# enkeejunior1/Diffusion-Pullback

Measured on AMD Instinct MI355X. Metric: pullback top-k SVD iters/sec (SD-v1.5 mid-block, 4x64x64), higher is better.
Workload: dtype bf16; 1 GPU; BASELINE configs[2]: SD-v1.5 4x64x64 latent, no edit prompt (seeded null ctx[1,77,768]), mid-block h[1280,8,8], t=696.27; pca_rank=5, ctx=null, samples_total=5, samples_this_rank=5, samples_advanced_together=1, spectrum=shaped (configs.Spectrum()), parallelism=single process, no collective, rccl_world_size=0, repeats=7

## Files before the change

diffusion_pullback_amd/csrc/attn_fused.hip:

```cpp
#include "kernels.h"

namespace dpb {

#ifndef DPB_ATT_ABL
#define DPB_ATT_ABL 0
#endif
#ifndef DPB_OUT_STORE_ATT
#define DPB_OUT_STORE_ATT 0
#endif
#define DPB_ATT_PAD 8

constexpr int att_waves(int d) { return d > 80 ? 4 : 8; }

template <int D, int W = att_waves(D)> struct FA {
  static constexpr int WAVES = W, NT = WAVES * 64;
  static constexpr int NS = (D + 15) / 16;
  static constexpr int DP = NS * 16;
  static constexpr int ND = (D + 31) / 32;
  static constexpr int DO = ND * 32;
  static constexpr int BI = D <= 80 ? 128 : 64;
  static constexpr int LDR = (DP > DO ? DP : DO) + DPB_ATT_PAD;
  static constexpr int LDT = BI + 4;
  static constexpr int ROW_ELEMS = BI * LDR;
  static constexpr int T_ELEMS = DO * LDT;
// ... 14 lines not shown
}
template <int D, int NTH = FA<D>::NT>
__device__ inline void commit_row(const RowRegs<D, NTH>& rg, bf16* lds, int tid) {
  using F = FA<D>;
  constexpr int CPR = F::DP / 8, N = (F::BI * CPR + NTH - 1) / NTH;
#pragma unroll
  for (int i = 0; i < N; ++i) {
    const int c = tid + i * NTH;
    if (c < F::BI * CPR) *reinterpret_cast<uint4*>(lds + (c / CPR) * F::LDR + (c % CPR) * 8) = rg.v[i];
  }
}
template <int D, int NTH = FA<D>::NT> struct TRegs { uint4 v[(FA<D>::DO * (FA<D>::BI / 8) + NTH - 1) / NTH]; };
template <int D, int NTH = FA<D>::NT>
__device__ inline void fetch_t(const bf16* __restrict__ src, long gs, TRegs<D, NTH>& rg, int tid) {
  using F = FA<D>;
  constexpr int CPR = F::BI / 8, N = (F::DO * CPR + NTH - 1) / NTH;
#pragma unroll
  for (int i = 0; i < N; ++i) {
    const int c = tid + i * NTH;
    const int r = c / CPR, cc = (c % CPR) * 8;
    rg.v[i] = make_uint4(0, 0, 0, 0);
    if (c < F::DO * CPR && r < D) rg.v[i] = *reinterpret_cast<const uint4*>(src + (long)r * gs + cc);
  }
}
template <int D, int NTH = FA<D>::NT>
__device__ inline void commit_t(const TRegs<D, NTH>& rg, bf16* lds, int tid) {
  using F = FA<D>;
  constexpr int CPR = F::BI / 8, N = (F::DO * CPR + NTH - 1) / NTH;
#pragma unroll
  for (int i = 0; i < N; ++i) {
    const int c = tid + i * NTH;
    if (c < F::DO * CPR) {
      bf16* dst = lds + (c / CPR) * F::LDT + (c % CPR) * 8;
      *reinterpret_cast<uint2*>(dst) = make_uint2(rg.v[i].x, rg.v[i].y);
      *reinterpret_cast<uint2*>(dst + 4) = make_uint2(rg.v[i].z, rg.v[i].w);
    }
  }
}
template <int D>
__device__ inline void load_outer_frags(const bf16* __restrict__ rowptr, bf16x8* f, int lhi) {
  using F = FA<D>;
#pragma unroll
  for (int st = 0; st < F::NS; ++st) {
    const int col = st * 16 + lhi * 8;
    uint4 v = make_uint4(0, 0, 0, 0);
    if (col < D) v = *reinterpret_cast<const uint4*>(rowptr + col);
    f[st] = *reinterpret_cast<bf16x8*>(&v);
  }
}
__device__ inline bf16x8 lds_a_frag(const bf16* tile, int row, int ld, int col) {
  return *reinterpret_cast<const bf16x8*>(tile + row * ld + col);
}
__device__ inline bf16x8 lds_t_frag(const bf16* tile, int drow, int ld, int base, int lhi) {
  uint2 lo = *reinterpret_cast<const uint2*>(tile + drow * ld + base + 4 * lhi);
  uint2 hi = *reinterpret_cast<const uint2*>(tile + drow * ld + base + 8 + 4 * lhi);
  uint4 v = make_uint4(lo.x, lo.y, hi.x, hi.y);
  return *reinterpret_cast<bf16x8*>(&v);
}
typedef __attribute__((ext_vector_type(4))) short short4_;
__device__ inline bf16x8 lds_tr_frag(const bf16* tile, int ld, int base, int d0, int lane) {
  const int i16 = lane & 15, g = lane >> 4;
  const bf16* p = tile + (base + 4 * (g >> 1) + (i16 >> 2)) * ld + d0 + (g & 1) * 16 + (i16 & 3) * 4;
  short4_ lo = __builtin_amdgcn_ds_read_tr16_b64_v4i16((__attribute__((address_space(3))) short4_*)p);
  short4_ hi = __builtin_amdgcn_ds_read_tr16_b64_v4i16((__attribute__((address_space(3))) short4_*)(p + 8 * ld));
  uint2 l2 = *reinterpret_cast<uint2*>(&lo), h2 = *reinterpret_cast<uint2*>(&hi);
  uint4 v = make_uint4(l2.x, l2.y, h2.x, h2.y);
  return *reinterpret_cast<bf16x8*>(&v);
}
template <int FL>
__device__ inline void pack_b(const float* x, bf16x8* out) {
  out[0] = H16<FL>::pack8(x);
  out[1] = H16<FL>::pack8(x + 8);
}
struct BlockXY { int x, y; };
__device__ inline BlockXY xcd_group_blocks(int on) {
  const int nx = gridDim.x, ny = gridDim.y;
  if (!on || (ny & 7)) return {(int)blockIdx.x, (int)blockIdx.y};
  const int lin = blockIdx.y * nx + blockIdx.x, xcd = lin & 7, slot = lin >> 3;
  return {slot % nx, (slot / nx) * 8 + xcd};
}

static int g_attn_shared = getenv("DPB_ATTN_SHARED") ? atoi(getenv("DPB_ATTN_SHARED")) : 2;
void attn_debug_shared(int bits) { g_attn_shared = bits; }

#define MFMA(a, b, c) H16<FL>::mfma(a, b, c)

struct FusedArgs {
  const bf16 *Q, *K, *V, *O;
  const bf16 *KT, *VT, *QT;
  const float* stats;
  float* Drow;
  float* Dout;
  const bf16 *dQ, *dK, *dV, *dVT;
  bf16* dO;
  const bf16 *gO, *gOT;
  bf16 *gQ, *gK, *gV;
  int accQ, accK, accV;
  int xcd;
  int L, C, Co, H, kps;
  float scale;
};

template <int D, int FL, int W = att_waves(D)>
__global__ __launch_bounds__((FA<D, W>::NT)) void attn_fwd_kernel(FusedArgs a, bf16* O, float* stats_out) {
  using F = FA<D, W>;
  __shared__ __attribute__((aligned(16))) bf16 sm[2 * F::ROW_ELEMS];
  bf16* sK = sm; bf16* sV = sK + F::ROW_ELEMS;
  const int tid = threadIdx.x, lane = tid & 63, wave = tid >> 6, l31 = lane & 31, lhi = lane >> 5;
  const BlockXY blk = xcd_group_blocks(a.xcd);
  const int b = blk.y / a.H, h = blk.y % a.H;
  const int q_ = blk.x * (F::WAVES * 32) + wave * 32 + l31;
  const bool live = q_ < a.L;
  const int q = live ? q_ : a.L - 1;
  const long LC = (long)a.L * a.C;
  const bf16* Kp = a.K + b * LC + h * D;
  const bf16* Vp = a.V + b * LC + h * D;
  bf16x8 qf[F::NS];
  load_outer_frags<D>(a.Q + b * LC + (long)q * a.C + h * D, qf, lhi);
  const float c2 = a.scale * 1.44269504088896f;
  constexpr float FWD_THR = 4.f;
  constexpr bool LSUM = F::DP > D;
  constexpr unsigned ONE16 = FL ? 0x3C00u : 0x3F80u, VONE = LSUM ? ONE16 : 0u;
  f32x16 acc[F::ND];
#pragma unroll
  for (int d = 0; d < F::ND; ++d)
#pragma unroll
    for (int r = 0; r < 16; ++r) acc[d][r] = 0.f;
  float m = -INFINITY, l = 0.f;
  RowRegs<D, F::NT> rK, rV;
  fetch_row<D, F::NT>(Kp, a.C, rK, tid); fetch_row<D, F::NT, VONE>(Vp, a.C, rV, tid);
  for (int k0 = 0; k0 < a.L; k0 += F::BI) {
    __syncthreads();
    commit_row<D, F::NT>(rK, sK, tid); commit_row<D, F::NT>(rV, sV, tid);
    __syncthreads();
    if (k0 + F::BI < a.L) {
      const int k1 = k0 + F::BI;
      fetch_row<D, F::NT>(Kp + (long)k1 * a.C, a.C, rK, tid); fetch_row<D, F::NT, VONE>(Vp + (long)k1 * a.C, a.C, rV, tid);
    }
#pragma unroll
    for (int kb = 0; kb < F::BI / 32; ++kb) {
      f32x16 s;
#pragma unroll
      for (int r = 0; r < 16; ++r) s[r] = 0.f;
#pragma unroll
      for (int stp = 0; stp < F::NS; ++stp) s = MFMA(lds_a_frag(sK, kb * 32 + l31, F::LDR, stp * 16 + lhi * 8), qf[stp], s);
      float mx = s[0];
#pragma unroll
      for (int r = 1; r < 16; ++r) mx = fmaxf(mx, s[r]);
      mx = fmaxf(mx, __shfl_xor(mx, 32, 64)) * c2;
      if (!__all(mx - m <= FWD_THR)) {
        const float mn = fmaxf(m, mx);
        const float alpha = __builtin_amdgcn_exp2f(m - mn);
#pragma unroll
        for (int d = 0; d < F::ND; ++d)
#pragma unroll
          for (int r = 0; r < 16; ++r) acc[d][r] *= alpha;
        if (!LSUM) l *= alpha;
        m = mn;
      }
      float p[16];
#pragma unroll
      for (int r = 0; r < 16; ++r) p[r] = __builtin_amdgcn_exp2f(__builtin_fmaf(s[r], c2, -m));
      if (!LSUM) {
        float ps = 0.f;
#pragma unroll
        for (int r = 0; r < 16; ++r) ps += p[r];
// ... 92 lines not shown
        kf[stp] = lds_a_frag(sK, kb * 32 + l31, F::LDR, stp * 16 + lhi * 8);
        dkf[stp] = lds_a_frag(sdK, kb * 32 + l31, F::LDR, stp * 16 + lhi * 8);
      }
    };
    if constexpr (PIPE) load1(0);
#pragma unroll
    for (int kb = 0; kb < F::BI / 32; ++kb) {
      bf16x8 vf[2][F::ND], dvf[2][F::ND];
      if constexpr (PIPE) {
#pragma unroll
        for (int ks = 0; ks < 2; ++ks)
#pragma unroll
          for (int d = 0; d < F::ND; ++d) {
            vf[ks][d] = lds_tr_frag(sV, F::LDR, kb * 32 + ks * 16, d * 32, lane);
            dvf[ks][d] = lds_tr_frag(sdV, F::LDR, kb * 32 + ks * 16, d * 32, lane);
          }
        __builtin_amdgcn_sched_barrier(0);
      } else {
        load1(kb);
      }
      f32x16 s, ds;
#pragma unroll
      for (int r = 0; r < 16; ++r) s[r] = ds[r] = 0.f;
#pragma unroll
      for (int stp = 0; stp < F::NS; ++stp) {
        s = MFMA(kf[stp], qf[stp], s);
        ds = MFMA(kf[stp], dqf[stp], ds);
        if (!((DPB_ATT_ABL & 2) && D == 40 && stp == F::NS - 1)) ds = MFMA(dkf[stp], qf[stp], ds);
      }
      if constexpr (PIPE) {
        __builtin_amdgcn_sched_barrier(0);
        if (kb + 1 < F::BI / 32) load1(kb + 1);
        __builtin_amdgcn_sched_barrier(0);
      }
      float p[16], x[16];
#pragma unroll
      for (int r = 0; r < 16; ++r) {
        p[r] = (DPB_ATT_ABL & 4) ? c2 * s[r] - m2 : __builtin_amdgcn_exp2f(c2 * s[r] - m2);
        x[r] = p[r] * (a.scale * ds[r]);
        if constexpr (!SUMROW) delta += x[r];
      }
      bf16x8 pb[2], xb[2];
      pack_b<FL>(p, pb);
      pack_b<FL>(x, xb);
#pragma unroll
      for (int ks = 0; ks < 2; ++ks)
#pragma unroll
        for (int d = 0; d < F::ND; ++d) {
          if constexpr (!PIPE) {
            vf[ks][d] = lds_tr_frag(sV, F::LDR, kb * 32 + ks * 16, d * 32, lane);
            dvf[ks][d] = lds_tr_frag(sdV, F::LDR, kb * 32 + ks * 16, d * 32, lane);
          }
          if ((DPB_ATT_ABL & 1) && D == 40 && ks == 1 && d == 1) continue;
          acc[d] = MFMA(vf[ks][d], xb[ks], acc[d]);
          acc[d] = MFMA(dvf[ks][d], pb[ks], acc[d]);
        }
    }
  }
  if constexpr (SUMROW) delta = __shfl(acc[D / 32][((D % 32) & 3) + 4 * ((D % 32) >> 3)], l31, 64);
  else delta += __shfl_xor(delta, 32, 64);
  const long LCo = (long)a.L * a.Co;
  const bf16* Op = a.O + b * LCo + (long)q * a.Co + h * D;
  bf16* dOp = a.dO + j * LCo + (long)q * a.Co + h * D;
#pragma unroll
  for (int d = 0; d < F::ND; ++d)
#pragma unroll
    for (int g = 0; g < 4; ++g) {
      const int col = d * 32 + 8 * g + 4 * lhi;
      if (col < D && live) {
        uint2 ov = *reinterpret_cast<const uint2*>(Op + col);
        unsigned ow[2] = {ov.x, ov.y};
        unsigned w[2];
#pragma unroll
        for (int i = 0; i < 2; ++i) {
          float o0 = H16<FL>::lo(ow[i]), o1 = H16<FL>::hi(ow[i]);
          float v0 = acc[d][g * 4 + 2 * i] - delta * o0, v1 = acc[d][g * 4 + 2 * i + 1] - delta * o1;
          w[i] = H16<FL>::pack2(v0, v1);
        }
        store_out8<DPB_OUT_STORE_ATT>(dOp + col, w[0], w[1]);
      }
    }
}

template <int D, int FL>
__global__ __launch_bounds__(FA<D>::NT) void attn_adj_q_kernel(FusedArgs a) {
  using F = FA<D>;
  __shared__ __attribute__((aligned(16))) bf16 sm[2 * F::ROW_ELEMS];
  bf16* sK = sm; bf16* sV = sK + F::ROW_ELEMS;
  const int tid = threadIdx.x, lane = tid & 63, wave = tid >> 6, l31 = lane & 31, lhi = lane >> 5;
  const BlockXY blk = xcd_group_blocks(a.xcd);
  const int j = blk.y / a.H, h = blk.y % a.H, b = j / a.kps;
  const int q_ = blk.x * (F::WAVES * 32) + wave * 32 + l31;
  const bool live = q_ < a.L;
  const int q = live ? q_ : a.L - 1;
  const long LC = (long)a.L * a.C;
  const bf16* Kp = a.K + b * LC + h * D;
  const bf16* Vp = a.V + b * LC + h * D;
  bf16x8 qf[F::NS], gof[F::NS], of[F::NS];
  load_outer_frags<D>(a.Q + b * LC + (long)q * a.C + h * D, qf, lhi);
  const long LCo = (long)a.L * a.Co;
  load_outer_frags<D>(a.gO + j * LCo + (long)q * a.Co + h * D, gof, lhi);
  load_outer_frags<D>(a.O + b * LCo + (long)q * a.Co + h * D, of, lhi);
  float Dq = 0.f;
#pragma unroll
  for (int stp = 0; stp < F::NS; ++stp) {
    const unsigned short* g16 = reinterpret_cast<const unsigned short*>(&gof[stp]);
    const unsigned short* o16 = reinterpret_cast<const unsigned short*>(&of[stp]);
#pragma unroll
    for (int e = 0; e < 8; ++e) Dq += H16<FL>::up(g16[e]) * H16<FL>::up(o16[e]);
  }
  Dq += __shfl_xor(Dq, 32, 64);
  const float* st = a.stats + (((long)b * a.H + h) * a.L + q) * 2;
  const float c2 = a.scale * 1.44269504088896f;
  const float m2 = st[0] * 1.44269504088896f - __builtin_log2f(st[1]);
  f32x16 acc[F::ND];
#pragma unroll
  for (int d = 0; d < F::ND; ++d)
#pragma unroll
    for (int r = 0; r < 16; ++r) acc[d][r] = 0.f;
  RowRegs<D> rK, rV;
  fetch_row<D>(Kp, a.C, rK, tid); fetch_row<D>(Vp, a.C, rV, tid);
  for (int k0 = 0; k0 < a.L; k0 += F::BI) {
    __syncthreads();
    commit_row<D>(rK, sK, tid); commit_row<D>(rV, sV, tid);
    __syncthreads();
    if (k0 + F::BI < a.L) {
      const int k1 = k0 + F::BI;
      fetch_row<D>(Kp + (long)k1 * a.C, a.C, rK, tid); fetch_row<D>(Vp + (long)k1 * a.C, a.C, rV, tid);
    }
#pragma unroll
    for (int kb = 0; kb < F::BI / 32; ++kb) {
      f32x16 s, gp;
#pragma unroll
      for (int r = 0; r < 16; ++r) s[r] = gp[r] = 0.f;
#pragma unroll
      for (int stp = 0; stp < F::NS; ++stp) {
        s = MFMA(lds_a_frag(sK, kb * 32 + l31, F::LDR, stp * 16 + lhi * 8), qf[stp], s);
        gp = MFMA(lds_a_frag(sV, kb * 32 + l31, F::LDR, stp * 16 + lhi * 8), gof[stp], gp);
      }
      float gs[16];
#pragma unroll
      for (int r = 0; r < 16; ++r) gs[r] = __builtin_amdgcn_exp2f(c2 * s[r] - m2) * (gp[r] - Dq);
      bf16x8 gsb[2];
      pack_b<FL>(gs, gsb);
#pragma unroll
      for (int ks = 0; ks < 2; ++ks)
#pragma unroll
        for (int d = 0; d < F::ND; ++d)
          acc[d] = MFMA(lds_tr_frag(sK, F::LDR, kb * 32 + ks * 16, d * 32, lane), gsb[ks], acc[d]);
    }
  }
  bf16* gQp = a.gQ + j * LC + (long)q * a.C + h * D;
#pragma unroll
  for (int d = 0; d < F::ND; ++d)
#pragma unroll
    for (int g = 0; g < 4; ++g) {
      const int col = d * 32 + 8 * g + 4 * lhi;
      if (col < D && live) {
        float v[4];
#pragma unroll
        for (int i = 0; i < 4; ++i) v[i] = a.scale * acc[d][g * 4 + i];
        if (a.accQ) {
          uint2 ov = *reinterpret_cast<const uint2*>(gQp + col);
          v[0] += H16<FL>::lo(ov.x); v[1] += H16<FL>::hi(ov.x);
          v[2] += H16<FL>::lo(ov.y); v[3] += H16<FL>::hi(ov.y);
        }
// ... 611 lines not shown
}

static bool head_dim_ok(int d) { return d == 40 || d == 64 || d == 80 || d == 160; }
#define DPB_ATT_DISPATCH(d, fl, ...)                                                        \
  do {                                                                                       \
    if ((fl) == 0) { constexpr int FL = 0; DPB_ATT_D(d, __VA_ARGS__) } else { constexpr int FL = 1; DPB_ATT_D(d, __VA_ARGS__) } \
  } while (0)
#define DPB_ATT_D(d, ...)                                          \
  if ((d) == 40) { constexpr int D = 40; __VA_ARGS__; }            \
  else if ((d) == 64) { constexpr int D = 64; __VA_ARGS__; }       \
  else if ((d) == 80) { constexpr int D = 80; __VA_ARGS__; }       \
  else { constexpr int D = 160; __VA_ARGS__; }

int cross_attention_supported(int dtype, int d, int Lq, int Lk, int kv_const) {
  return dtype != DT_F32 && kv_const && head_dim_ok(d) && Lk <= XKEYS && Lq % 32 == 0 && (Lq >= 128 ? Lq % 128 == 0 : true);
}

int launch_attn_cross(const CrossAttnArgs& f, int nt, hipStream_t st) {
  CrossArgs a;
  a.Q = (const bf16*)f.Q; a.K = (const bf16*)f.K; a.V = (const bf16*)f.V; a.BT = (const bf16*)f.BT;
  a.X = (const bf16*)f.X; a.Y = (bf16*)f.Y;
  a.L = f.L; a.Lk = f.Lk; a.Lkp = f.Lkp; a.C = f.C; a.Ck = f.Ck; a.Cx = f.Cx; a.Cy = f.Cy; a.H = f.H; a.kps = f.kps;
  a.a_is_v = f.adjoint; a.accumulate = f.accumulate; a.scale = f.scale; a.xcd = 0;
  a.c_in = f.adjoint ? 1.f : f.scale; a.c_out = f.adjoint ? f.scale : 1.f;
  a.primal = f.primal; a.Pst = f.primal ? f.Pstash : nullptr;
  if (f.primal) { a.a_is_v = 0; a.c_in = 1.f; a.c_out = 1.f; a.accumulate = 0; }
  const int waves = f.L >= 128 ? 4 : f.L / 32;
  dim3 grid(f.L / (waves * 32), nt * f.H);
  if (!head_dim_ok(f.d)) { set_error("cross attention: head dim %d unsupported", f.d); return -1; }
  if (a.Pst) DPB_ATT_DISPATCH(f.d, f.fl, DPB_LAUNCH((attn_cross_kernel<D, FL, true>), grid, dim3(waves * 64), 0, st, a));
  else DPB_ATT_DISPATCH(f.d, f.fl, DPB_LAUNCH((attn_cross_kernel<D, FL>), grid, dim3(waves * 64), 0, st, a));
  DPB_CHECK(hipGetLastError());
  return 0;
}

int fused_attention_supported(int dtype, int d, int L, int kv_const) {
  return dtype != DT_F32 && !kv_const && head_dim_ok(d) && ((L >= 256 && L % (att_waves(d) * 32) == 0) || (d == 160 && L == 64));
}

static int attn_xcd_on() { static int on = getenv("DPB_ATTN_XCD") ? atoi(getenv("DPB_ATTN_XCD")) : 0; return on; }

static FusedArgs to_args(const FusedAttnArgs& f) {
  FusedArgs a;
  a.xcd = attn_xcd_on();
  a.Q = (const bf16*)f.Q; a.K = (const bf16*)f.K; a.V = (const bf16*)f.V; a.O = (const bf16*)f.O;
  a.KT = (const bf16*)f.KT; a.VT = (const bf16*)f.VT; a.QT = (const bf16*)f.QT; a.stats = f.stats; a.Drow = f.Drow; a.Dout = nullptr;
  a.dQ = (const bf16*)f.dQ; a.dK = (const bf16*)f.dK; a.dV = (const bf16*)f.dV; a.dVT = (const bf16*)f.dVT; a.dO = (bf16*)f.dO;
  a.gO = (const bf16*)f.gO; a.gOT = (const bf16*)f.gOT; a.gQ = (bf16*)f.gQ; a.gK = (bf16*)f.gK; a.gV = (bf16*)f.gV;
  a.accQ = f.accQ; a.accK = f.accK; a.accV = f.accV;
  a.L = f.L; a.C = f.C; a.Co = f.Co; a.H = f.H; a.kps = f.kps; a.scale = f.scale;
  return a;
}

int launch_attn_fwd_fused(const FusedAttnArgs& f, int batch, void* O, float* stats, hipStream_t st) {
  FusedArgs a = to_args(f);
  dim3 grid((f.L + att_waves(f.d) * 32 - 1) / (att_waves(f.d) * 32), batch * f.H);
  if (!head_dim_ok(f.d)) { set_error("fused attention: head dim %d unsupported", f.d); return -1; }
  static const int fwd4 = getenv("DPB_ATTN_FWD4") ? atoi(getenv("DPB_ATTN_FWD4")) : 1;
  if (fwd4 && att_waves(f.d) == 8 && f.L % 128 == 0 && f.L >= 256 && (long)grid.x * grid.y < 256) {
    dim3 g4(f.L / 128, batch * f.H);
    if (f.d == 40) { if (f.fl) DPB_LAUNCH((attn_fwd_kernel<40, 1, 4>), g4, dim3(256), 0, st, a, (bf16*)O, stats); else DPB_LAUNCH((attn_fwd_kernel<40, 0, 4>), g4, dim3(256), 0, st, a, (bf16*)O, stats); }
    else if (f.d == 64) { if (f.fl) DPB_LAUNCH((attn_fwd_kernel<64, 1, 4>), g4, dim3(256), 0, st, a, (bf16*)O, stats); else DPB_LAUNCH((attn_fwd_kernel<64, 0, 4>), g4, dim3(256), 0, st, a, (bf16*)O, stats); }
    else { if (f.fl) DPB_LAUNCH((attn_fwd_kernel<80, 1, 4>), g4, dim3(256), 0, st, a, (bf16*)O, stats); else DPB_LAUNCH((attn_fwd_kernel<80, 0, 4>), g4, dim3(256), 0, st, a, (bf16*)O, stats); }
    DPB_CHECK(hipGetLastError());
    return 0;
  }
  DPB_ATT_DISPATCH(f.d, f.fl, DPB_LAUNCH((attn_fwd_kernel<D, FL>), grid, dim3(att_waves(D) * 64), 0, st, a, (bf16*)O, stats));
  DPB_CHECK(hipGetLastError());
  return 0;
}

static int att_block_waves(int d, int L, int pairs) {
  static const int force = getenv("DPB_ATTN_WAVES") ? atoi(getenv("DPB_ATTN_WAVES")) : 0;
  if (d != 40 || L % 256) return att_waves(d);
  if (force == 4 || force == 8) return force;
  return ((long)(L / 256) * pairs) % 256 == 0 ? 8 : 4;
}

int attn_jvp_block_waves(int d, int L, int pairs) { return att_block_waves(d, L, pairs); }

int launch_attn_jvp_fused(const FusedAttnArgs& f, int nt, hipStream_t st) {
  FusedArgs a = to_args(f);
  if (!head_dim_ok(f.d)) { set_error("fused attention: head dim %d unsupported", f.d); return -1; }
  if (att_block_waves(f.d, f.L, nt * f.H) == 4 && f.d == 40) {
    dim3 g4(f.L / 128, nt * f.H);
    if (f.fl) DPB_LAUNCH((attn_jvp_kernel<40, 1, 4>), g4, dim3(256), 0, st, a);
    else DPB_LAUNCH((attn_jvp_kernel<40, 0, 4>), g4, dim3(256), 0, st, a);
    DPB_CHECK(hipGetLastError());
    return 0;
  }
  dim3 grid((f.L + att_waves(f.d) * 32 - 1) / (att_waves(f.d) * 32), nt * f.H);
  DPB_ATT_DISPATCH(f.d, f.fl, DPB_LAUNCH((attn_jvp_kernel<D, FL>), grid, dim3(att_waves(D) * 64), 0, st, a));
  DPB_CHECK(hipGetLastError());
  return 0;
}

static int attn_adj_route(int d, int L, int kps, int nt, bool have_drow) {
  static const int multi = getenv("DPB_ATTN_MULTI") ? atoi(getenv("DPB_ATTN_MULTI")) : 1;
  const int shared = g_attn_shared;
  const bool dsh = d == 40 || (d == 64 && (shared & 4));
  int r = 0;
  if (dsh && (multi & 1) && L % 128 == 0 && nt % kps == 0) r |= 1;
  if (dsh && (shared & 2) && L % 64 == 0 && kps >= 4 && nt % kps == 0 && have_drow) r |= 2;
  return r;
}
int attn_adj_route_bits(int d, int L, int kps, int nt) { return attn_adj_route(d, L, kps, nt, true); }

int launch_attn_adj_fused(const FusedAttnArgs& f, int nt, hipStream_t st) {
  FusedArgs a = to_args(f);
  dim3 grid((f.L + att_waves(f.d) * 32 - 1) / (att_waves(f.d) * 32), nt * f.H);
  if (!head_dim_ok(f.d)) { set_error("fused attention: head dim %d unsupported", f.d); return -1; }
  const int route = attn_adj_route(f.d, f.L, f.kps, nt, f.Drow != nullptr);
  if (route & 1) {
    constexpr int TJ = 5;
    const int ngrp = (f.kps + TJ - 1) / TJ;
    const dim3 gq(f.L / 128, (nt / f.kps) * f.H * ngrp);
    if (route & 2) a.Dout = a.Drow;
#define DPB_ADJQ(DV, FLV) DPB_LAUNCH((attn_adj_q_multi_kernel<DV, TJ, FLV>), gq, dim3(256), 0, st, a)
    if (f.d == 40) { if (f.fl) DPB_ADJQ(40, 1); else DPB_ADJQ(40, 0); }
    else { if (f.fl) DPB_ADJQ(64, 1); else DPB_ADJQ(64, 0); }
#undef DPB_ADJQ
  } else {
    DPB_ATT_DISPATCH(f.d, f.fl, DPB_LAUNCH((attn_adj_q_kernel<D, FL>), grid, dim3(att_waves(D) * 64), 0, st, a));
  }
  if (route & 2) {
    constexpr int TJ = 5;
    const int ngrp = (f.kps + TJ - 1) / TJ;
    const dim3 gs(f.L / 64, (nt / f.kps) * f.H * ngrp);
    const unsigned nrd = (unsigned)(((long)nt * f.L * f.H + 255) / 256);
#define DPB_ADJKV(DV, FLV)                                                                                                          \
    do {                                                                                                                              \
      if (!(route & 1)) DPB_LAUNCH((attn_rowdot_kernel<DV, FLV>), dim3(nrd), dim3(256), 0, st, a, nt);                              \
      DPB_LAUNCH((attn_adj_kv_shared_kernel<DV, TJ, FLV>), gs, dim3(SHK<DV, TJ>::NT), 0, st, a);                                    \
    } while (0)
    if (f.d == 40) { if (f.fl) DPB_ADJKV(40, 1); else DPB_ADJKV(40, 0); }
    else { if (f.fl) DPB_ADJKV(64, 1); else DPB_ADJKV(64, 0); }
#undef DPB_ADJKV
  } else if (att_block_waves(f.d, f.L, nt * f.H) == 4 && f.d == 40) {
    dim3 g4(f.L / 128, nt * f.H);
    if (f.fl) DPB_LAUNCH((attn_adj_kv_kernel<40, 1, 4>), g4, dim3(256), 0, st, a);
    else DPB_LAUNCH((attn_adj_kv_kernel<40, 0, 4>), g4, dim3(256), 0, st, a);
  } else {
    DPB_ATT_DISPATCH(f.d, f.fl, DPB_LAUNCH((attn_adj_kv_kernel<D, FL>), grid, dim3(att_waves(D) * 64), 0, st, a));
  }
  DPB_CHECK(hipGetLastError());
  return 0;
}

}
```

diffusion_pullback_amd/csrc/engine.cpp:

```cpp
#include <math.h>
#include <stdarg.h>
#include <stdio.h>
#include <stdlib.h>
#include <string.h>

#include <string>
#include <vector>

#include "../../include/dpb.h"
#include "kernels.h"

namespace dpb {

static thread_local char g_err[1024] = "";
void set_error(const char* fmt, ...) {
  va_list ap;
  va_start(ap, fmt);
  vsnprintf(g_err, sizeof(g_err), fmt, ap);
  va_end(ap);
}
const char* last_error() { return g_err; }
thread_local long launch_count = 0;

static inline size_t align_up(size_t v, size_t a = 256) { return (v + a - 1) / a * a; }
// ... 1732 lines not shown
int dpb_engine_profile(dpb_engine* e, int enable) {
  if (!e) return fail("null engine");
  for (auto& p : e->prof) { (void)hipEventDestroy(p.a); (void)hipEventDestroy(p.b); }
  e->prof.clear();
  e->profiling = enable != 0;
  if (e->profiling) {
    hipEvent_t a, b;
    DPB_CHECK(hipEventCreate(&a));
    DPB_CHECK(hipEventCreate(&b));
    float best = 1e9f;
    for (int i = 0; i < 24; ++i) {
      DPB_CHECK(hipEventRecord(a, e->stream));
      if (int r = launch_axpy(e->dtype, e->ws + e->zeros, e->ws + e->zeros, 64, 0, e->stream)) return r;
      DPB_CHECK(hipEventRecord(b, e->stream));
      DPB_CHECK(hipEventSynchronize(b));
      float ms = 0;
      DPB_CHECK(hipEventElapsedTime(&ms, a, b));
      if (i >= 4) best = ms < best ? ms : best;
    }
    (void)hipEventDestroy(a);
    (void)hipEventDestroy(b);
    best -= 1.5e-3f;
    if (best < 0.f) best = 0.f;
    e->prof_overhead_ms = best < 1e8f ? best : 0.f;
  }
  return 0;
}

int dpb_engine_profile_dump(dpb_engine* e, const char* path) {
  if (!e || !path) return fail("null argument");
  DPB_CHECK(hipStreamSynchronize(e->stream));
  FILE* f = fopen(path, "w");
  if (!f) return fail("cannot open %s", path);
  fprintf(f, "idx,big,gather,M,N,K,Z,us,tflops,raw_us,bracket_overhead_us\n");
  int i = 0;
  for (auto& p : e->prof) {
    float raw = 0;
    (void)hipEventElapsedTime(&raw, p.a, p.b);
    const float ms = raw > e->prof_overhead_ms ? raw - e->prof_overhead_ms : 0.f;
    fprintf(f, "%d,%d,%d,%d,%d,%d,%d,%.2f,%.2f,%.2f,%.2f\n", i++, p.big, p.gather, p.M, p.N, p.K, p.Z, ms * 1e3, ms > 0 ? p.flops / (ms * 1e-3) / 1e12 : 0.0,
            raw * 1e3, e->prof_overhead_ms * 1e3);
  }
  fclose(f);
  return 0;
}

int dpb_engine_profile_read(dpb_engine* e, int big_tile, int64_t* count, double* total_ms, double* flops) {
  if (!e || !count || !total_ms || !flops) return fail("null argument");
  DPB_CHECK(hipStreamSynchronize(e->stream));
  *count = 0; *total_ms = 0; *flops = 0;
  const bool raw = big_tile >= 1000;
  if (raw) big_tile -= 1000;
  if (big_tile < 0 || big_tile > 12) return fail("dpb_engine_profile_read: kind must be 0..12 or 1000..1012");
  for (auto& p : e->prof) {
    if (p.big != big_tile) continue;
    float ms = 0;
    DPB_CHECK(hipEventElapsedTime(&ms, p.a, p.b));
    if (!raw) ms = ms > e->prof_overhead_ms ? ms - e->prof_overhead_ms : 0.f;
    *count += 1; *total_ms += ms; *flops += p.flops;
  }
  return 0;
}

int dpb_engine_profile_overhead(const dpb_engine* e, double* bracket_overhead_ms) {
  if (!e || !bracket_overhead_ms) return fail("null argument");
  *bracket_overhead_ms = e->prof_overhead_ms;
  return 0;
}

int dpb_debug_set(const char* key, int value) {
  static int tile = 0, splitk = 0, kch = 0;
  if (!key) return fail("null key");
  if (!strcmp(key, "gemm_tile")) tile = value;
  else if (!strcmp(key, "gemm_splitk")) splitk = value;
  else if (!strcmp(key, "gemm_kch")) kch = value;
  else if (!strcmp(key, "gemm_dma_auto")) { gemm_debug_dma_auto(value); return 0; }
  else if (!strcmp(key, "gemm_order")) { gemm_debug_order(value); return 0; }
  else if (!strcmp(key, "p8")) { gemm_debug_p8(value); return 0; }
  else if (!strcmp(key, "halo_loop")) { conv_halo_debug_loop(value); return 0; }
  else if (!strcmp(key, "wres")) { gemm_debug_wres(value); return 0; }
  else if (!strcmp(key, "gn_deterministic")) { gn_debug_deterministic(value); return 0; }
  else if (!strcmp(key, "graph_iterate")) { g_graph_iterate = value; return 0; }
  else if (!strcmp(key, "attn_shared")) { attn_debug_shared(value); return 0; }
  else if (!strcmp(key, "lazy_reduce")) { g_lazy_reduce = value; return 0; }
  else if (!strcmp(key, "ln_fuse")) { g_ln_fuse = value; return 0; }
  else if (!strcmp(key, "cross_primal")) { g_cross_primal = value; return 0; }
  else if (!strcmp(key, "cross_fold")) { g_cross_fold = value; return 0; }
  else if (!strcmp(key, "geglu_fwd")) { g_geglu_fwd = value; return 0; }
  else if (!strcmp(key, "iter_alias")) { g_iter_alias = value; return 0; }
  else return fail("unknown debug key %s", key);
  gemm_debug_set(tile, splitk, kch);
  return 0;
}

int dpb_debug_gemm_plan(int dtype, int M, int N, int K, int conv_hw, int conv_cin, int epilogue, int64_t slab_bytes, int* kind, int* tile,
                        int* splitk) {
  if (!kind || !tile || !splitk) return fail("null argument");
  if (dtype != DPB_F32 && dtype != DPB_BF16 && dtype != DPB_F16) return fail("bad dtype %d", dtype);
  static char dummy[16];
  GemmArgs a;
  a.M = M; a.N = N; a.K = K; a.lda = K; a.ldb = K; a.ldc = N;
  a.zeros = dummy;
  if (slab_bytes > 0) { a.slab = (float*)dummy; a.slab_bytes = (size_t)slab_bytes; }
  a.epi = epilogue;
  if (epilogue == EPI_XATT) { a.xatt_p = (const float*)dummy; a.xatt_h = N / 128; a.xatt_lk = 77; a.ldc = 80 * a.xatt_h; a.C = dummy; }
  if (conv_hw > 0) {
    if (conv_cin <= 0 || K != 9 * conv_cin || M % (conv_hw * conv_hw)) return fail("conv plan: K must be 9*cin and M whole images");
    a.gather = GATHER_CONV; a.H = a.W = a.Ho = a.Wo = conv_hw; a.Cin = conv_cin; a.KS = 3; a.stride = 1; a.pad = 1; a.lda = conv_cin;
  }
  const GemmPlan pl = gemm_plan(dtype, a);
  if (!pl.row) return -1;
  *kind = pl.kind; *tile = pl.tile; *splitk = pl.splitk;
  return 0;
}

int dpb_debug_cross_fold(const dpb_engine* e, int index, int64_t* info) {
  if (!e || !info) return fail("null argument");
  int n = 0;
  for (size_t i = 0; i < e->ops.size(); ++i) {
    if (e->ops[i].d.kind != DPB_OP_ATTENTION || !e->plans[e->ops[i].attn].fold_ok) continue;
    if (n++ != index) continue;
    const AttnPlan& p = e->plans[e->ops[i].attn];
    const int64_t v[12] = {(int64_t)i, p.fold_live, p.heads * p.d, p.heads, p.Lq, p.Lk, (int64_t)p.Gt, (int64_t)p.Gk, (int64_t)p.F, (int64_t)p.Fk, (int64_t)p.Pf, (int64_t)e->S1};
    memcpy(info, v, sizeof(v));
    return 0;
  }
  return fail("dpb_debug_cross_fold: the tape has %d layers that can take the folded route, index %d", n, index);
}

int dpb_engine_stats(const dpb_engine* e, int64_t* launches, double* gemm_flops, double* gemm_bytes) {
  if (!e) return fail("null engine");
  if (launches) *launches = e->n_launch;
  if (gemm_flops) *gemm_flops = e->flops;
  if (gemm_bytes) *gemm_bytes = e->gbytes;
  return 0;
}

}
```

diffusion_pullback_amd/csrc/kernels.h:

```cpp
#pragma once
#include <algorithm>
#include <cstdarg>
#include <cstdio>
#include <type_traits>
#include <utility>

#include "common.h"

namespace dpb {

enum { GATHER_NONE = 0, GATHER_CONV = 1, GATHER_CONVT = 2, GATHER_UPCONV = 3 };
enum { EPI_PLAIN = 0, EPI_GEGLU_TAN = 1, EPI_GEGLU_ADJ = 2, EPI_LN_TAN = 3, EPI_LN_ADJ = 4, EPI_GEGLU_FWD = 5, EPI_XATT = 6 };
struct GemmArgs {
  const void* A = nullptr; const void* B = nullptr; void* C = nullptr; const void* R = nullptr;
  const float* bias = nullptr;
  const void* rowbias = nullptr;
  int rows_per_sample = 1, rowbias_div = 1;
  int ldrb = 0;
  int M = 0, N = 0, K = 0;
  int lda = 0, ldb = 0, ldc = 0, ldr = 0;
  int Z1 = 1, Z2 = 1;
  long sA1 = 0, sA2 = 0, sB1 = 0, sB2 = 0, sC1 = 0, sC2 = 0, sR1 = 0, sR2 = 0;
  int divA = 1, divB = 1;
  float alpha = 1.f;
// ... 119 lines not shown
void gn_debug_deterministic(int on);
int gn_deterministic();
bool gemm_wres_supported(int dtype, const GemmArgs& a);
int launch_gemm_wres(const GemmArgs& a, hipStream_t st);
void gemm_debug_wres(int on);
void gemm_debug_p8(int on);
void gemm_debug_order(int o);

enum { MODE_PRIMAL = 0, MODE_TANGENT = 1, MODE_ADJOINT = 2 };
struct SlabSrc {
  const float* slab = nullptr; int splitk = 0; long MN = 0; int N = 0;
  const void* R = nullptr; int ldr = 0;
  void* store = nullptr;
};
struct GNArgs {
  const void* x = nullptr;
  const void* d = nullptr;
  void* y = nullptr;
  const float* gamma = nullptr; const float* beta = nullptr;
  int astride = 0;
  double* pstats = nullptr;
  double* tstats = nullptr;
  float* part = nullptr;
  size_t part_bytes = 0;
  int* ticket = nullptr;
  int det = 1;
  int red = 0;
  int Bp = 1, NT = 0, kps = 1;
  int HW = 0, C = 0, G = 32;
  float eps = 1e-5f;
  int silu = 0, accumulate = 0;
  SlabSrc src;
};
int launch_groupnorm(int dtype, int mode, const GNArgs& a, hipStream_t st);
constexpr int ADAGN_MAX_OPS = 32;
struct AdaGNTable { const float* gamma[ADAGN_MAX_OPS]; const float* beta[ADAGN_MAX_OPS]; const void* emb[ADAGN_MAX_OPS]; float* og[ADAGN_MAX_OPS]; float* ob[ADAGN_MAX_OPS]; int C[ADAGN_MAX_OPS]; };
struct AdaGNOp { const float* gamma; const float* beta; const void* emb; float* og; float* ob; int C; };
int launch_adagn_affine(int dtype, const AdaGNOp* ops, int nops, long ld, int batch, int per_sample, hipStream_t st);
bool groupnorm_is_one_launch(int dtype, const GNArgs& a);

struct LNArgs {
  const void* x = nullptr; const void* d = nullptr; void* y = nullptr;
  const float* gamma = nullptr; const float* beta = nullptr;
  int rows_per_sample = 0, Bp = 1, NT = 0, kps = 1, C = 0;
  float eps = 1e-5f;
  int accumulate = 0;
  SlabSrc src;
};
int launch_layernorm(int dtype, int mode, const LNArgs& a, hipStream_t st);

int launch_softmax_fwd(int dtype, void* S, long Z, int Lq, int Lk, int ld, int causal, hipStream_t st);
int launch_softmax_jvp(int dtype, const void* P, void* dS, float* D, long Z, int Z2, int kps, int Lq, int Lk, int ld,
                       hipStream_t st);
int launch_softmax_adjT(int dtype, const void* PT, void* gPT, const float* D, long Z, int Z2, int kps, int Lk, int Lq,
                        int ld, hipStream_t st);
int launch_transpose(int dtype, const void* in, void* out, int Z1, int Z2, long s1, long s2, int R, int Ccols, int ldin,
                     int ldout, long outZstride, hipStream_t st);

struct FusedAttnArgs {
  const void *Q = nullptr, *K = nullptr, *V = nullptr, *O = nullptr, *KT = nullptr, *VT = nullptr, *QT = nullptr;
  const float* stats = nullptr;
  float* Drow = nullptr;
  const void *dQ = nullptr, *dK = nullptr, *dV = nullptr, *dVT = nullptr; void* dO = nullptr;
  const void *gO = nullptr, *gOT = nullptr; void *gQ = nullptr, *gK = nullptr, *gV = nullptr;
  int accQ = 0, accK = 0, accV = 0;
  int fl = 0;
  int L = 0, C = 0, Co = 0, H = 0, d = 0, kps = 1;
  float scale = 1.f;
};
int fused_attention_supported(int dtype, int d, int L, int kv_const);
void attn_debug_shared(int bits);
struct CrossAttnArgs {
  const void *Q = nullptr, *K = nullptr, *V = nullptr;
  const void* BT = nullptr;
  const void* X = nullptr; void* Y = nullptr;
  int L = 0, Lk = 0, Lkp = 0, C = 0, Ck = 0, Cx = 0, Cy = 0, H = 0, d = 0, kps = 1, adjoint = 0, accumulate = 0, fl = 0;
  int primal = 0;
  float* Pstash = nullptr;
  float scale = 1.f;
};
int cross_attention_supported(int dtype, int d, int Lq, int Lk, int kv_const);
int launch_attn_cross(const CrossAttnArgs& f, int nt, hipStream_t st);
int attn_adj_route_bits(int d, int L, int kps, int nt);
int attn_jvp_block_waves(int d, int L, int pairs);
int launch_attn_fwd_fused(const FusedAttnArgs& f, int batch, void* O, float* stats, hipStream_t st);
int launch_attn_jvp_fused(const FusedAttnArgs& f, int nt, hipStream_t st);
int launch_attn_adj_fused(const FusedAttnArgs& f, int nt, hipStream_t st);

struct GegluArgs {
  const void* h = nullptr;
  const void* d = nullptr;
  void* y = nullptr;
  int rows_per_sample = 0, Bp = 1, NT = 0, kps = 1, F = 0;
  int accumulate = 0;
  int stash = 1;
  int il = 0;
};
int launch_geglu(int dtype, int mode, const GegluArgs& a, hipStream_t st);
int launch_silu(int dtype, const void* x, void* y, long n, hipStream_t st);
int launch_quick_gelu(int dtype, const void* x, void* y, long n, hipStream_t st);
int launch_gelu(int dtype, const void* x, void* y, long n, hipStream_t st);
int launch_embed_tokens(int dtype, const int* ids, const void* tok, const void* pos, float* out, int batch, int L, int C, int vocab, hipStream_t st);
int launch_axpy(int dtype, const void* x, void* y, long n, int accumulate, hipStream_t st);
int launch_copy_cols(int dtype, const void* src, int lds, int cs0, void* dst, int ldd, int cd0, long rows, int ncols,
                     int accumulate, hipStream_t st);
int launch_zero_cols(int dtype, void* dst, int ldd, int cd0, long rows, int ncols, hipStream_t st);
int launch_nchw_to_nhwc(int dtype, const float* src, void* dst, int n, int C, int HW, int Cpad, hipStream_t st);
int launch_nhwc_to_nchw(int dtype, const void* src, float* dst, int n, int C, int HW, int Cpad, hipStream_t st);
constexpr int SHIFT_MAX_ROWS = 64;
struct ShiftRows { int dir[SHIFT_MAX_ROWS]; float scale[SHIFT_MAX_ROWS]; };
int launch_shift_tap(int dtype, void* h, const float* u, const int* dir, const float* scale, int batch, int bcast, int C, int Cv, long HW,
                     hipStream_t st);
constexpr int REPL_MAX_BUFS = 32;
struct ReplTable { void* p[REPL_MAX_BUFS]; long chunks[REPL_MAX_BUFS]; };
int launch_replicate_rows(void* const* bufs, const size_t* sample_bytes, int nbufs, int batch, hipStream_t st);
int launch_pool2x2_sum(int dtype, const void* in, void* out, int n, int H, int W, int C, int accumulate, hipStream_t st);
int launch_pool2x2(int dtype, const void* in, void* out, int n, int H, int W, int C, float scale, int accumulate, hipStream_t st);
int launch_up2x2(int dtype, const void* in, void* out, int n, int H, int W, int C, float scale, int accumulate, hipStream_t st);

struct OrthArgs {
  const float* W = nullptr;
  const float* Vprev = nullptr;
  float* V = nullptr;
  float* s = nullptr;
  float* conv = nullptr;
  double* scratch = nullptr;
  size_t scratch_bytes = 0;
  int k = 0; long N = 0;
  int batch = 1; long stride_w = 0, stride_v = 0, stride_s = 0, stride_conv = 0; size_t scratch_stride = 0;
};
constexpr int ORTH_MAX_RANK = 128;
int launch_orth(const OrthArgs& a, hipStream_t st);
size_t orth_scratch_bytes(int k, long N);

const char* pca_invalid(int q, long N, long D);
size_t pca_scratch_bytes(int q, long N, long D);
int launch_pca_lowrank(const float* H, long N, long D, const float* R, int q, int niter, float* u, float* s, void* scratch, size_t scratch_bytes,
                       hipStream_t st);

struct ScratchCarver {
  size_t off = 0;
  size_t take(size_t bytes) { const size_t o = off; off += (bytes + 255) / 256 * 256; return o; }
};
__attribute__((format(printf, 5, 6))) inline int check_scratch(const char* who, const void* scratch, size_t have, size_t need, const char* sizer, ...) {
  if ((uintptr_t)scratch % 256) { set_error("%s: scratch must be 256-byte aligned", who); return -1; }
  if (have >= need) return 0;
  char call[160];
  va_list ap;
  va_start(ap, sizer);
  vsnprintf(call, sizeof(call), sizer, ap);
  va_end(ap);
  set_error("%s: scratch of %zu bytes, %s = %zu needed", who, have, call, need);
  return -1;
}
#define DPB_BY_RANK(k, ...)                                                \
  do {                                                                     \
    if ((k) <= 16) { constexpr int KM = 16, NT = 256; __VA_ARGS__; }       \
    else if ((k) <= 32) { constexpr int KM = 32, NT = 1024; __VA_ARGS__; } \
    else { constexpr int KM = 64, NT = 1024; __VA_ARGS__; }                \
  } while (0)
#define DPB_BY_RANK128(k, ...)                                             \
  do {                                                                     \
    if ((k) <= 64) DPB_BY_RANK(k, __VA_ARGS__);                            \
    else { constexpr int KM = 128, NT = 1024; __VA_ARGS__; }               \
  } while (0)
#define DPB_BY_TILES(k, ...)                                   \
// ... 72 lines not shown
```

Baseline: 121.9 iters/s.

## Add paired-tangent fused attention JVP kernel sharing K/V tiles and softmax

Adds an attention JVP kernel for head dim 40 in which each block advances two tangent directions of the same sample. They share the staged K/V tiles, the QK^T scores and the exponentiated probabilities, while each tangent keeps its own dK/dV tiles in LDS. The delta term is taken from an appended ones column in the V tile instead of a separate reduction, and an odd leftover tangent runs through a single-tangent variant. This is meant to remove redundant K/V loads and exp work across tangents. In exchange it uses more LDS and registers per block, which may lower occupancy.

Measured after the change: 122.5 iters/s (median of 6 runs). Within noise of the previous version (+0.5%).

```diff
diff --git a/diffusion_pullback_amd/csrc/attn_fused.hip b/diffusion_pullback_amd/csrc/attn_fused.hip
--- a/diffusion_pullback_amd/csrc/attn_fused.hip
+++ b/diffusion_pullback_amd/csrc/attn_fused.hip
@@ -120,6 +120,8 @@
 
 static int g_attn_shared = getenv("DPB_ATTN_SHARED") ? atoi(getenv("DPB_ATTN_SHARED")) : 2;
 void attn_debug_shared(int bits) { g_attn_shared = bits; }
+static int g_attn_jvp_pair = getenv("DPB_ATTN_JVP_PAIR") ? atoi(getenv("DPB_ATTN_JVP_PAIR")) : 3;
+int attn_debug_jvp_pair(int bits) { const int was = g_attn_jvp_pair; if (bits >= 0) g_attn_jvp_pair = bits; return was; }
 
 #define MFMA(a, b, c) H16<FL>::mfma(a, b, c)
 
@@ -378,6 +380,179 @@
     }
 }
 
+template <int D, int BI, int NTH> struct RowRegs2 { uint4 v[(2 * BI * (FA<D>::DP / 8) + NTH - 1) / NTH]; };
+template <int D, int BI, int NTH, unsigned ONE1 = 0>
+__device__ inline void fetch_row2(const bf16* __restrict__ src0, const bf16* __restrict__ src1, int gs, RowRegs2<D, BI, NTH>& rg, int tid, int wave) {
+  constexpr int CPR = FA<D>::DP / 8, T = BI * CPR, N = (2 * T + NTH - 1) / NTH;
+  static_assert(T % 64 == 0, "the tile of a chunk must be wave-uniform");
+#pragma unroll
+  for (int i = 0; i < N; ++i) {
+    const int c2 = tid + i * NTH;
+    const bool second = wave * 64 + i * NTH >= T;
+    const int c = second ? c2 - T : c2;
+    const int r = c / CPR, cc = (c % CPR) * 8;
+    rg.v[i] = make_uint4(ONE1 != 0 && second && cc == D ? ONE1 : 0u, 0, 0, 0);
+    if (c2 < 2 * T && cc < D) rg.v[i] = *reinterpret_cast<const uint4*>((second ? src1 : src0) + (unsigned)(r * gs + cc));
+  }
+}
+template <int D, int BI, int NTH>
+__device__ inline void commit_row2(const RowRegs2<D, BI, NTH>& rg, bf16* lds0, bf16* lds1, int tid, int wave) {
+  constexpr int CPR = FA<D>::DP / 8, T = BI * CPR, N = (2 * T + NTH - 1) / NTH;
+#pragma unroll
+  for (int i = 0; i < N; ++i) {
+    const int c2 = tid + i * NTH;
+    const bool second = wave * 64 + i * NTH >= T;
+    const int c = second ? c2 - T : c2;
+    if (c2 < 2 * T) *reinterpret_cast<uint4*>((second ? lds1 : lds0) + (c / CPR) * FA<D>::LDR + (c % CPR) * 8) = rg.v[i];
+  }
+}
+
+constexpr int JVP_PAIR_BI = 64;
+
+template <int D, int FL, int W, bool TWO>
+__device__ __forceinline__ void attn_jvp_pair_body(const FusedArgs& a, bf16* sm, int bx, int jA, int b, int h) {
+  using F = FA<D, W>;
+  constexpr int BI = JVP_PAIR_BI, NT = F::NT, TILE = BI * F::LDR;
+  static_assert(F::DO > D && ((D % 32) & 4) == 0 && F::DP > D, "the pair kernel takes delta from the ones column of the V tile");
+  bf16* sK = sm; bf16* sV = sK + TILE; bf16* sdKA = sV + TILE; bf16* sdVA = sdKA + TILE; bf16* sdKB = sdVA + TILE; bf16* sdVB = sdKB + TILE;
+  const int tid = threadIdx.x, lane = tid & 63, wave = tid >> 6, l31 = lane & 31, lhi = lane >> 5;
+  const int jB = jA + (TWO ? 1 : 0);
+  const int q_ = bx * (F::WAVES * 32) + wave * 32 + l31;
+  const bool live = q_ < a.L;
+  const int q = live ? q_ : a.L - 1;
+  const long LC = (long)a.L * a.C;
+  const bf16* Kp = a.K + b * LC + h * D;
+  const bf16* Vp = a.V + b * LC + h * D;
+  const bf16* dKAp = a.dK + jA * LC + h * D;
+  const bf16* dVAp = a.dV + jA * LC + h * D;
+  const bf16* dKBp = a.dK + jB * LC + h * D;
+  const bf16* dVBp = a.dV + jB * LC + h * D;
+  bf16x8 qf[F::NS], dqfA[F::NS], dqfB[F::NS];
+  load_outer_frags<D>(a.Q + b * LC + h * D + (long)q * a.C, qf, lhi);
+  load_outer_frags<D>(a.dQ + jA * LC + h * D + (long)q * a.C, dqfA, lhi);
+  if constexpr (TWO) load_outer_frags<D>(a.dQ + jB * LC + h * D + (long)q * a.C, dqfB, lhi);
+  const float* st = a.stats + (((long)b * a.H + h) * a.L + q) * 2;
+  const float c2 = a.scale * 1.44269504088896f;
+  const float m2 = st[0] * 1.44269504088896f - __builtin_log2f(st[1]);
+  constexpr unsigned VONE = FL ? 0x3C00u : 0x3F80u;
+  f32x16 accA[F::ND], accB[F::ND];
+#pragma unroll
+  for (int d = 0; d < F::ND; ++d)
+#pragma unroll
+    for (int r = 0; r < 16; ++r) accA[d][r] = accB[d][r] = 0.f;
+  const int wu = __builtin_amdgcn_readfirstlane(wave);
+  RowRegs2<D, BI, NT> rKV, rdA, rdB;
+  auto fetch = [&](int k1) {
+    fetch_row2<D, BI, NT, VONE>(Kp + (long)k1 * a.C, Vp + (long)k1 * a.C, a.C, rKV, tid, wu);
+    fetch_row2<D, BI, NT>(dKAp + (long)k1 * a.C, dVAp + (long)k1 * a.C, a.C, rdA, tid, wu);
+    if constexpr (TWO) fetch_row2<D, BI, NT>(dKBp + (long)k1 * a.C, dVBp + (long)k1 * a.C, a.C, rdB, tid, wu);
+  };
+  fetch(0);
+  for (int k0 = 0; k0 < a.L; k0 += BI) {
+    __syncthreads();
+    commit_row2<D, BI, NT>(rKV, sK, sV, tid, wu);
+    commit_row2<D, BI, NT>(rdA, sdKA, sdVA, tid, wu);
+    if constexpr (TWO) commit_row2<D, BI, NT>(rdB, sdKB, sdVB, tid, wu);
+    __syncthreads();
+    if (k0 + BI < a.L) fetch(k0 + BI);
+#pragma unroll
+    for (int kb = 0; kb < BI / 32; ++kb) {
+      bf16x8 kf[F::NS], vf[2][F::ND];
+#pragma unroll
+      for (int stp = 0; stp < F::NS; ++stp) kf[stp] = lds_a_frag(sK, kb * 32 + l31, F::LDR, stp * 16 + lhi * 8);
+      f32x16 s;
+#pragma unroll
+      for (int r = 0; r < 16; ++r) s[r] = 0.f;
+#pragma unroll
+      for (int stp = 0; stp < F::NS; ++stp) s = MFMA(kf[stp], qf[stp], s);
+#pragma unroll
+      for (int ks = 0; ks < 2; ++ks)
+#pragma unroll
+        for (int d = 0; d < F::ND; ++d) vf[ks][d] = lds_tr_frag(sV, F::LDR, kb * 32 + ks * 16, d * 32, lane);
+      float p[16];
+#pragma unroll
+      for (int r = 0; r < 16; ++r) p[r] = __builtin_amdgcn_exp2f(c2 * s[r] - m2);
+      bf16x8 pb[2];
+      pack_b<FL>(p, pb);
+      auto tangent = [&](const bf16* sdK, const bf16* sdV, const bf16x8* dqf, f32x16* acc) {
+        bf16x8 dkf[F::NS], dvf[2][F::ND];
+#pragma unroll
+        for (int stp = 0; stp < F::NS; ++stp) dkf[stp] = lds_a_frag(sdK, kb * 32 + l31, F::LDR, stp * 16 + lhi * 8);
+        f32x16 ds;
+#pragma unroll
+        for (int r = 0; r < 16; ++r) ds[r] = 0.f;
+#pragma unroll
+        for (int stp = 0; stp < F::NS; ++stp) {
+          ds = MFMA(kf[stp], dqf[stp], ds);
+          ds = MFMA(dkf[stp], qf[stp], ds);
+        }
+#pragma unroll
+        for (int ks = 0; ks < 2; ++ks)
+#pragma unroll
+          for (int d = 0; d < F::ND; ++d) dvf[ks][d] = lds_tr_frag(sdV, F::LDR, kb * 32 + ks * 16, d * 32, lane);
+        float x[16];
+#pragma unroll
+        for (int r = 0; r < 16; ++r) x[r] = p[r] * (a.scale * ds[r]);
+        bf16x8 xb[2];
+        pack_b<FL>(x, xb);
+#pragma unroll
+        for (int ks = 0; ks < 2; ++ks)
+#pragma unroll
+          for (int d = 0; d < F::ND; ++d) {
+            acc[d] = MFMA(vf[ks][d], xb[ks], acc[d]);
+            acc[d] = MFMA(dvf[ks][d], pb[ks], acc[d]);
+          }
+      };
+      tangent(sdKA, sdVA, dqfA, accA);
+      if constexpr (TWO) {
+        __builtin_amdgcn_sched_barrier(0);
+        tangent(sdKB, sdVB, dqfB, accB);
+      }
+    }
+  }
+  const long LCo = (long)a.L * a.Co;
+  const bf16* Op = a.O + b * LCo + (long)q * a.Co + h * D;
+  auto finish = [&](const f32x16* acc, int j) {
+    const float delta = __shfl(acc[D / 32][((D % 32) & 3) + 4 * ((D % 32) >> 3)], l31, 64);
+    bf16* dOp = a.dO + j * LCo + (long)q * a.Co + h * D;
+#pragma unroll
+    for (int d = 0; d < F::ND; ++d)
+#pragma unroll
+      for (int g = 0; g < 4; ++g) {
+        const int col = d * 32 + 8 * g + 4 * lhi;
+        if (col < D && live) {
+          uint2 ov = *reinterpret_cast<const uint2*>(Op + col);
+          unsigned ow[2] = {ov.x, ov.y};
+          unsigned w[2];
+#pragma unroll
+          for (int i = 0; i < 2; ++i) {
+            float o0 = H16<FL>::lo(ow[i]), o1 = H16<FL>::hi(ow[i]);
+            float v0 = acc[d][g * 4 + 2 * i] - delta * o0, v1 = acc[d][g * 4 + 2 * i + 1] - delta * o1;
+            w[i] = H16<FL>::pack2(v0, v1);
+          }
+          store_out8<DPB_OUT_STORE_ATT>(dOp + col, w[0], w[1]);
+        }
+      }
+  };
+  finish(accA, jA);
+  if constexpr (TWO) finish(accB, jB);
+}
+
+template <int D, int FL, int W>
+__global__ __launch_bounds__((FA<D, W>::NT), (W == 4 ? 2 : 1)) void attn_jvp_pair_kernel(FusedArgs a) {
+  __shared__ __attribute__((aligned(16))) bf16 sm[6 * JVP_PAIR_BI * FA<D, W>::LDR];
+  const BlockXY blk = xcd_group_blocks(a.xcd);
+  const int npair = a.kps >> 1, gps = (a.kps + 1) >> 1;
+  const int nb = (int)gridDim.y / (a.H * gps), ypair = nb * npair * a.H;
+  if (blk.y < ypair) {
+    const int g = blk.y / a.H, b = g / npair;
+    attn_jvp_pair_body<D, FL, W, true>(a, sm, blk.x, b * a.kps + 2 * (g % npair), b, blk.y % a.H);
+  } else {
+    const int y = blk.y - ypair, b = y / a.H;
+    attn_jvp_pair_body<D, FL, W, false>(a, sm, blk.x, b * a.kps + a.kps - 1, b, y % a.H);
+  }
+}
+
 template <int D, int FL>
 __global__ __launch_bounds__(FA<D>::NT) void attn_adj_q_kernel(FusedArgs a) {
   using F = FA<D>;
@@ -1155,7 +1330,15 @@
 int launch_attn_jvp_fused(const FusedAttnArgs& f, int nt, hipStream_t st) {
   FusedArgs a = to_args(f);
   if (!head_dim_ok(f.d)) { set_error("fused attention: head dim %d unsupported", f.d); return -1; }
-  if (att_block_waves(f.d, f.L, nt * f.H) == 4 && f.d == 40) {
+  const int waves = att_block_waves(f.d, f.L, nt * f.H);
+  if (f.d == 40 && f.kps >= 2 && nt % f.kps == 0 && f.L % (waves * 32) == 0 && (g_attn_jvp_pair & (waves == 4 ? 1 : 2))) {
+    dim3 gp(f.L / (waves * 32), (nt / f.kps) * ((f.kps + 1) / 2) * f.H);
+    if (waves == 4) { if (f.fl) DPB_LAUNCH((attn_jvp_pair_kernel<40, 1, 4>), gp, dim3(256), 0, st, a); else DPB_LAUNCH((attn_jvp_pair_kernel<40, 0, 4>), gp, dim3(256), 0, st, a); }
+    else { if (f.fl) DPB_LAUNCH((attn_jvp_pair_kernel<40, 1, 8>), gp, dim3(512), 0, st, a); else DPB_LAUNCH((attn_jvp_pair_kernel<40, 0, 8>), gp, dim3(512), 0, st, a); }
+    DPB_CHECK(hipGetLastError());
+    return 0;
+  }
+  if (waves == 4 && f.d == 40) {
     dim3 g4(f.L / 128, nt * f.H);
     if (f.fl) DPB_LAUNCH((attn_jvp_kernel<40, 1, 4>), g4, dim3(256), 0, st, a);
     else DPB_LAUNCH((attn_jvp_kernel<40, 0, 4>), g4, dim3(256), 0, st, a);
diff --git a/diffusion_pullback_amd/csrc/engine.cpp b/diffusion_pullback_amd/csrc/engine.cpp
--- a/diffusion_pullback_amd/csrc/engine.cpp
+++ b/diffusion_pullback_amd/csrc/engine.cpp
@@ -1838,6 +1838,7 @@
   else if (!strcmp(key, "gn_deterministic")) { gn_debug_deterministic(value); return 0; }
   else if (!strcmp(key, "graph_iterate")) { g_graph_iterate = value; return 0; }
   else if (!strcmp(key, "attn_shared")) { attn_debug_shared(value); return 0; }
+  else if (!strcmp(key, "attn_jvp_pair")) { return attn_debug_jvp_pair(value); }
   else if (!strcmp(key, "lazy_reduce")) { g_lazy_reduce = value; return 0; }
   else if (!strcmp(key, "ln_fuse")) { g_ln_fuse = value; return 0; }
   else if (!strcmp(key, "cross_primal")) { g_cross_primal = value; return 0; }
diff --git a/diffusion_pullback_amd/csrc/kernels.h b/diffusion_pullback_amd/csrc/kernels.h
--- a/diffusion_pullback_amd/csrc/kernels.h
+++ b/diffusion_pullback_amd/csrc/kernels.h
@@ -225,6 +225,7 @@
 int cross_attention_supported(int dtype, int d, int Lq, int Lk, int kv_const);
 int launch_attn_cross(const CrossAttnArgs& f, int nt, hipStream_t st);
 int attn_adj_route_bits(int d, int L, int kps, int nt);
+int attn_debug_jvp_pair(int bits);
 int attn_jvp_block_waves(int d, int L, int pairs);
 int launch_attn_fwd_fused(const FusedAttnArgs& f, int batch, void* O, float* stats, hipStream_t st);
 int launch_attn_jvp_fused(const FusedAttnArgs& f, int nt, hipStream_t st);
```
